# khanhha/temporal_inverse_kinematics

Measured on NVIDIA B200. Metric: IK-solved frames/sec (ST-GCN fwd + SMPL-X FK), higher is better.
Workload: dtype bf16

## Files before the change

include/tik.h:

```cpp
#ifndef TIK_H_
#define TIK_H_

#include <stdint.h>

#ifdef __cplusplus
extern "C" {
#endif

#define TIK_OK 0
#define TIK_ERR_INVALID (-1)
#define TIK_ERR_CUDA (-2)
#define TIK_ERR_UNSUPPORTED (-3)
#define TIK_ERR_WORKSPACE (-4)

#define TIK_F32 0
#define TIK_BF16 1

#define TIK_MAX_BLOCKS 16
#define TIK_MAX_SLABS 6
#define TIK_MAX_JOINTS 64

int tik_version(void);
const char* tik_last_error(void);
int tik_check_device(void);
// ... 16 lines not shown
int tik_stem_gcn(int dtype, const float* x_dev, const float* in_scale_dev, const float* in_shift_dev,
                 const float* agg_dev, const float* w_dev, const float* bias_dev, void* out_dev,
                 const float* res_w_dev, void* res_out_dev, int res_stride,
                 int64_t N, int T, int V, int Cin, int K, int Cout, int relu, void* stream);

typedef struct TikWindowing {
  int64_t frames;
  int32_t offset, stride, root_a, root_b;
} TikWindowing;

int tik_aggregate(int dtype, const void* x_dev, const float* agg_dev, void* out_dev,
                  int64_t N, int T, int V, int C, int K, void* stream);

int tik_gcn_fused(const void* x_dev, const void* abd_dev, const void* w_dev, const float* bias_dev, void* out_dev,
                  int64_t N, int T, int V, int Cin, int Cout, int relu, void* stream);

typedef struct TikSlab {
  const void* a_dev;
  int32_t c;
  int32_t t_in;
  int32_t t_mul;
  int32_t t_off;
} TikSlab;

#define TIK_ACT_NONE 0
#define TIK_ACT_RELU 1
#define TIK_ACT_LEAKY 2
#define TIK_RES_NONE 0
#define TIK_RES_IDENTITY 1
#define TIK_RES_STEM 2
// ... 127 lines not shown
```

temporal_inverse_kinematics_b200/_lib.py:

```python
import ctypes as C
import os

_HERE = os.path.dirname(os.path.abspath(__file__))
LIB_PATH = os.environ.get("TIK_LIB_PATH") or os.path.join(_HERE, "libtik.so")

HEADER_PATH = os.path.join(os.path.dirname(_HERE), "include", "tik.h")


def _header_defines():
    import re
    out = {}
    with open(HEADER_PATH) as f:
        for m in re.finditer(r"^#define\s+(TIK_\w+)\s+\(?(-?\d+)\)?", f.read(), re.M):
            out[m.group(1)] = int(m.group(2))
    return out


_H = _header_defines()
TIK_F32, TIK_BF16 = _H["TIK_F32"], _H["TIK_BF16"]
MAX_BLOCKS, MAX_SLABS, MAX_JOINTS = _H["TIK_MAX_BLOCKS"], _H["TIK_MAX_SLABS"], _H["TIK_MAX_JOINTS"]
ACT_NONE, ACT_RELU, ACT_LEAKY = 0, 1, 2
RES_NONE, RES_IDENTITY, RES_STEM, RES_CONV = 0, 1, 2, 3
OUT_NODE_MAJOR, OUT_TIME_MAJOR, OUT_ROWS_F32 = 0, 1, 2

# ... 49 lines not shown
    "tik_last_error": (C.c_char_p, []),
    "tik_check_device": (C.c_int, []),
    "tik_rot6d_to_rotmat": (C.c_int, [vp, vp, i64, vp]),
    "tik_aa_to_rotmat": (C.c_int, [vp, vp, i64, vp]),
    "tik_batch_rodrigues": (C.c_int, [vp, vp, i64, vp]),
    "tik_rotmat_to_aa": (C.c_int, [vp, vp, i64, C.c_int, vp]),
    "tik_quat_to_rotmat": (C.c_int, [vp, vp, i64, vp]),
    "tik_rotmat_to_quat": (C.c_int, [vp, vp, i64, vp]),
    "tik_quat_to_aa": (C.c_int, [vp, vp, i64, vp]),
    "tik_fk_body": (C.c_int, [vp, C.c_int, C.POINTER(f32), C.POINTER(i32), C.c_int, vp, vp, vp, vp, i64, vp]),
    "tik_stem_gcn": (C.c_int, [C.c_int, vp, vp, vp, vp, vp, vp, vp, vp, vp, C.c_int, i64, C.c_int, C.c_int, C.c_int,
                               C.c_int, C.c_int, C.c_int, vp]),
    "tik_aggregate": (C.c_int, [C.c_int, vp, vp, vp, i64, C.c_int, C.c_int, C.c_int, C.c_int, vp]),
    "tik_rowgemm": (C.c_int, [C.c_int, C.POINTER(TikRowGemm), vp]),
    "tik_gcn_fused": (C.c_int, [vp, vp, vp, vp, vp, i64, C.c_int, C.c_int, C.c_int, C.c_int, C.c_int, vp]),
    "tik_pack_bn": (C.c_int, [C.POINTER(TikRawBN), i64, vp, vp, vp]),
    "tik_pack_block_bytes": (C.c_int, [C.POINTER(TikRawBlock), C.c_int, C.c_int, C.POINTER(i64)]),
    "tik_pack_block": (C.c_int, [C.POINTER(TikRawBlock), C.c_int, C.c_int, C.POINTER(TikRawBN), C.POINTER(TikPackBuffers),
                                 C.POINTER(TikBlock), vp]),
    "tik_stgcn_out_frames": (C.c_int, [C.POINTER(TikNet), C.c_int]),
    "tik_stgcn_workspace_bytes": (C.c_int, [C.POINTER(TikNet), C.c_int, i64, i64, C.c_int, C.POINTER(i64)]),
    "tik_stgcn_plan_create": (C.c_int, [C.POINTER(TikNet), C.c_int, i64, i64, C.c_int, vp, i64, C.POINTER(vp)]),
    "tik_stgcn_plan_run": (C.c_int, [vp, vp, i64, vp, vp, vp]),
    "tik_stgcn_plan_run_windows": (C.c_int, [vp, vp, C.POINTER(TikWindowing), i64, vp, vp, vp]),
    "tik_stgcn_plan_profile": (C.c_int, [vp, vp, i64, vp, vp, C.POINTER(C.c_double), C.POINTER(i64), C.POINTER(C.c_double)]),
    "tik_stgcn_plan_launches": (i64, [vp, i64]),
    "tik_stgcn_plan_destroy": (None, [vp]),
    "tik_stgcn_latency_workspace_bytes": (C.c_int, [C.POINTER(TikNet), i64, C.c_int, C.POINTER(i64)]),
    "tik_stgcn_latency_create": (C.c_int, [C.POINTER(TikNet), i64, C.c_int, vp, i64, C.POINTER(vp)]),
    "tik_stgcn_latency_run": (C.c_int, [vp, vp, i64, vp, vp]),
# ... 63 lines not shown
```

temporal_inverse_kinematics_b200/build.py:

```python
import os
import shutil
import subprocess
import sys

HERE = os.path.dirname(os.path.abspath(__file__))
CSRC = os.path.join(HERE, "csrc")
LIB = os.path.join(HERE, "libtik.so")
SOURCES = ["geometry.cu", "fk.cu", "stem.cu", "stem_block.cu", "stgcn_simt.cu", "rowgemm_tf32.cu", "stgcn_umma.cu", "gcn_fused.cu", "tcn_halo.cu", "plan.cu", "latency.cu", "pack.cu"]
HEADERS = ["tik_common.cuh", "umma_prepared.h", "umma_ptx.cuh", os.path.join("..", "..", "include", "tik.h")]


def _nvcc():
    for c in (os.environ.get("NVCC"), shutil.which("nvcc"), "/usr/local/cuda/bin/nvcc"):
        if c and os.path.exists(c):
            return c
    raise RuntimeError("nvcc not found")


STAMP = os.path.join(HERE, "build", "flavour.txt")


def _flavour():
    if os.environ.get("TIK_TEST_WAIT") == "1":
        return "probe-testwait" if os.environ.get("TIK_PROBE") == "1" else "testwait"
# ... 58 lines not shown
```

temporal_inverse_kinematics_b200/csrc/plan.cu:

```cuda
#include <stdlib.h>
#include <string.h>

#include <algorithm>
#include <vector>

#include "tik_common.cuh"
#include "umma_prepared.h"

namespace tik {

static thread_local char g_err[512] = "";

bool pdl_enabled() {
  static int v = -1;
  if (v < 0) v = getenv("TIK_NO_PDL") ? 0 : 1;
  return v != 0;
}

LaunchOpts& launch_opts() {
  static thread_local LaunchOpts o = {0, 0};
  return o;
}
static int serpentine_enabled() {
  const char* e = getenv("TIK_SERPENTINE");
  return e ? atoi(e) : 1;
}
static int l2_hint_enabled() {
  const char* e = getenv("TIK_L2_HINT");
  return e ? atoi(e) : 0;
}

void set_error(const char* fmt, ...) {
  va_list ap;
  va_start(ap, fmt);
  vsnprintf(g_err, sizeof(g_err), fmt, ap);
  va_end(ap);
}

static int out_frames(int t, int stride) { return (t - 1) / stride + 1; }
static int64_t align_up(int64_t v, int64_t a) { return (v + a - 1) / a * a; }

struct Step {
  enum Kind { STEM = 0, AGG = 1, GEMM = 2, FUSED_GCN = 3, STEM_BLOCK = 4, TCN_HALO = 5 } kind;
  GcnFusedPrepared* fused = nullptr;
  StemBlockPrepared* stem_block = nullptr;
  TcnHaloPrepared* halo = nullptr;
  double fused_flops_per_clip = 0;
  TikRowGemm g;
  UmmaPrepared* prep = nullptr;
  const void* src = nullptr;
  void* dst = nullptr;
  void* dst2 = nullptr;
  int t = 0, c = 0;
  const TikBlock* blk = nullptr;
  bool out_is_feat = false;
  bool out_is_poses = false;
  bool agg_only = false;
  int k_identity = 0;
  const float* w_big = nullptr;
  const float* w_small = nullptr;
};
// ... 6 lines not shown
  int64_t n_chunk, n_max;
  int T, T_out;
  size_t es;
  std::vector<tik::Step> chunk_steps, batch_steps;
  uint8_t* feat = nullptr;
  int64_t feat_elems_per_clip = 0;
  int c_last = 0;
  ~TikPlan() {
    for (auto* v : {&chunk_steps, &batch_steps})
      for (auto& s : *v)
      {
        if (s.prep) tik::umma_free(s.prep);
        if (s.fused) tik::gcn_fused_free(s.fused);
        if (s.stem_block) tik::stem_block_free(s.stem_block);
        if (s.halo) tik::tcn_halo_free(s.halo);
      }
  }
};

namespace tik {

struct WsLayout {
  int64_t off_x0, off_x1, off_agg, off_h, off_r0, off_feat, off_z, off_abd, off_w16, off_eye, off_zbias, off_wsplit, total_bytes;
};

static int check_net(const TikNet* net, int dtype) {
  TIK_CHECK_ARG(net != nullptr, "null net");
  TIK_CHECK_ARG(dtype == TIK_F32 || dtype == TIK_BF16, "bad dtype %d", dtype);
  TIK_CHECK_ARG(net->n_blocks >= 1 && net->n_blocks <= TIK_MAX_BLOCKS, "n_blocks=%d", net->n_blocks);
  TIK_CHECK_ARG(net->V >= 1 && net->V <= 32 && net->K >= 1 && net->K <= 5, "V=%d K=%d unsupported", net->V, net->K);
// ... 55 lines not shown
  L->off_zbias = off; off = align_up(off + 32 * 128 * 4, 1024);
  L->off_wsplit = off;
  if (dtype == TIK_F32) {
    int64_t w_elems = 0;
    for (int i = 0; i < net->n_blocks; ++i) {
      const TikBlock& b = net->blocks[i];
      if (b.c_out <= 64) w_elems += align_up((int64_t)b.c_out * net->K * b.c_in, 256) + align_up((int64_t)b.c_out * (b.kt * b.c_out + b.c_in), 256);
    }
    if (net->head_hidden > 0 && net->head_hidden <= 64) w_elems += align_up((int64_t)net->head_hidden * V * net->blocks[net->n_blocks - 1].c_out, 256);
    if (net->head_hidden > 0 && net->head_out <= 64) w_elems += align_up((int64_t)net->head_out * net->head_hidden, 256);
    off = align_up(off + 2 * w_elems * 4, 1024);
  }
  L->total_bytes = off;
}

static int run_step(TikPlan* P, Step& st, const float* xc, int64_t n, int64_t clip_off, float* poses, cudaStream_t s,
                    const TikWindowing* win = nullptr, int64_t win_n0 = 0) {
  const TikNet& net = P->net;
  const int V = net.V;
  if (st.kind == Step::STEM) {
    const TikBlock& b = *st.blk;
    return stem_gcn_impl(P->dtype, xc, net.in_scale_dev, net.in_shift_dev, b.agg_dev, reinterpret_cast<const float*>(b.w_gcn_dev),
                         b.b_gcn_dev, st.dst, st.dst2 ? b.w_res_stem_dev : nullptr, st.dst2, b.stride, n, st.t, V, b.c_in, net.K,
                         b.c_out, 1, win, win_n0, s);
  }
  if (st.kind == Step::AGG) {
    return tik_aggregate(P->dtype, st.src, st.blk->agg_dev, st.dst, P->n_chunk, st.t, V, st.c, net.K, s);
  }
  if (st.kind == Step::FUSED_GCN) return gcn_fused_launch(st.fused, n, s);
  if (st.kind == Step::STEM_BLOCK) return stem_block_launch(st.stem_block, xc, n, win, win_n0, s);
  if (st.kind == Step::TCN_HALO) return tcn_halo_launch(st.halo, n * V, s);
  TikRowGemm g = st.g;
  if (g.v == 1) {
    g.t_out = (int32_t)(n * P->T_out);
    g.slabs[0].t_in = g.t_out;
  } else {
    g.nv = n * V;
  }
  if (st.out_is_feat) g.out_dev = P->feat + clip_off * P->feat_elems_per_clip * (int64_t)P->es;
  if (st.out_is_poses) g.out_dev = poses;
  return P->dtype == TIK_BF16 ? umma_launch(st.prep, &g, s) : rowgemm_f32_presplit(&g, st.w_big, st.w_small, s);
}

static int run_impl(TikPlan* P, const float* x, int64_t N, float* poses, void* feat_out, cudaStream_t s,
                    std::vector<cudaEvent_t>* events, std::vector<std::pair<Step*, int64_t>>* trace,
                    const TikWindowing* win = nullptr) {
// ... 114 lines not shown
  for (int i = 0; i < net->n_blocks; ++i) {
    const TikBlock& b = P->net.blocks[i];
    const int pad = (b.kt - 1) / 2;
    const int t_o = out_frames(t, b.stride);
    const bool last = i == net->n_blocks - 1;
    if (i == 0 && net->n_blocks > 1 && stem_block_supported(net, dtype) && !getenv("TIK_NO_STEM_BLOCK")) {
      Step s; s.kind = Step::STEM_BLOCK; s.blk = &b; s.t = t;
      int rcs = stem_block_prepare(&P->net, ws + L.off_w16, xbuf[0], n_chunk, t, &s.stem_block);
      if (rcs != TIK_OK) { delete P; return rcs; }
      s.fused_flops_per_clip = 2.0 * V * t * (double)b.c_out * (K * b.c_in + b.kt * b.c_out + (b.res_kind == TIK_RES_STEM ? b.c_in : 0));
      P->chunk_steps.push_back(s);
      cur = 0;
      t = t_o;
      continue;
    }
    if (i == 0) {
      Step s; s.kind = Step::STEM; s.dst = hbuf; s.t = t; s.blk = &b;
      s.dst2 = b.res_kind == TIK_RES_STEM ? r0buf : nullptr;
      P->chunk_steps.push_back(s);
    } else if (dtype == TIK_BF16 && gcn_fused_supported(b.c_in, b.c_out, V, K) && !getenv("TIK_NO_FUSED_GCN")) {
      const int f = gcn_fused_frames(t, b.c_in);
      std::vector<float> a_host((size_t)V * V);
      cudaError_t ce = cudaMemcpy(a_host.data(), b.agg_dev, a_host.size() * sizeof(float), cudaMemcpyDeviceToHost);
      std::vector<__nv_bfloat16> abd_host(128 * 128, __float2bfloat16_rn(0.f));
      for (int w = 0; w < V; ++w)
        for (int v = 0; v < V; ++v)
          for (int q = 0; q < f; ++q) abd_host[(size_t)(w * f + q) * 128 + (v * f + q)] = __float2bfloat16_rn(a_host[(size_t)v * V + w]);
      void* abd_dev = ws + L.off_abd + (int64_t)i * 128 * 128 * 2;
      if (ce == cudaSuccess) ce = cudaMemcpy(abd_dev, abd_host.data(), abd_host.size() * 2, cudaMemcpyHostToDevice);
      if (ce != cudaSuccess) { set_error("plan: Abd upload failed: %s", cudaGetErrorString(ce)); delete P; return TIK_ERR_CUDA; }
      Step s; s.kind = Step::FUSED_GCN; s.blk = &b; s.t = t;
      int rcf = gcn_fused_prepare(xbuf[cur], abd_dev, b.w_gcn_dev, b.b_gcn_dev, hbuf, n_chunk, t, V, b.c_in, b.c_out, 1, &s.fused);
      if (rcf != TIK_OK) { delete P; return rcf; }
      s.fused_flops_per_clip = 2.0 * V * t * (double)b.c_in * b.c_out;
      P->chunk_steps.push_back(s);
    } else {
      const bool tc_agg = dtype == TIK_BF16 && K == 1 && b.c_in % 128 == 0 && gcn_fused_supported(128, 128, V, 1) &&
                          !getenv("TIK_NO_FUSED_GCN") && !getenv("TIK_NO_TC_AGG");
      if (tc_agg) {
        const int f = gcn_fused_frames(t);
        std::vector<float> a_host((size_t)V * V);
        cudaError_t ce = cudaMemcpy(a_host.data(), b.agg_dev, a_host.size() * sizeof(float), cudaMemcpyDeviceToHost);
        std::vector<__nv_bfloat16> abd_host(128 * 128, __float2bfloat16_rn(0.f)), eye_host(128 * 128, __float2bfloat16_rn(0.f));
        for (int w = 0; w < V; ++w)
          for (int v = 0; v < V; ++v)
            for (int q = 0; q < f; ++q) abd_host[(size_t)(w * f + q) * 128 + (v * f + q)] = __float2bfloat16_rn(a_host[(size_t)v * V + w]);
        for (int d = 0; d < 128; ++d) eye_host[(size_t)d * 128 + d] = __float2bfloat16_rn(1.f);
        void* abd_dev = ws + L.off_abd + (int64_t)i * 128 * 128 * 2;
        if (ce == cudaSuccess) ce = cudaMemcpy(abd_dev, abd_host.data(), abd_host.size() * 2, cudaMemcpyHostToDevice);
        if (ce == cudaSuccess) ce = cudaMemcpy(ws + L.off_eye, eye_host.data(), eye_host.size() * 2, cudaMemcpyHostToDevice);
        if (ce == cudaSuccess) ce = cudaMemset(ws + L.off_zbias, 0, 32 * 128 * 4);
        if (ce != cudaSuccess) { set_error("plan: aggregation operands upload failed: %s", cudaGetErrorString(ce)); delete P; return TIK_ERR_CUDA; }
        for (int c0 = 0; c0 < b.c_in; c0 += 128) {
          Step s; s.kind = Step::FUSED_GCN; s.blk = &b; s.t = t; s.agg_only = true;
          int rcf = gcn_fused_prepare(reinterpret_cast<uint8_t*>(xbuf[cur]) + (size_t)c0 * 2, abd_dev, ws + L.off_eye,
                                      reinterpret_cast<const float*>(ws + L.off_zbias), reinterpret_cast<uint8_t*>(agg) + (size_t)c0 * 2,
                                      n_chunk, t, V, 128, 128, 0, &s.fused, b.c_in, b.c_in);
          if (rcf != TIK_OK) { delete P; return rcf; }
          P->chunk_steps.push_back(s);
        }
      } else {
        Step s; s.kind = Step::AGG; s.src = xbuf[cur]; s.dst = agg; s.t = t; s.c = b.c_in; s.blk = &b;
        P->chunk_steps.push_back(s);
      }
// ... 125 lines not shown
  TIK_CHECK_ARG(P->net.head_hidden == 0 || poses, "poses pointer required");
  std::vector<cudaEvent_t> ev;
  std::vector<std::pair<Step*, int64_t>> trace;
  cudaStream_t s = (cudaStream_t)stream;
  int rc = run_impl(P, x, N, poses, nullptr, s, &ev, &trace);
  if (rc != TIK_OK) return rc;
  TIK_CUDA(cudaStreamSynchronize(s));
  for (int k = 0; k < 3; ++k) { ms_by_kind[k] = 0; launches_by_kind[k] = 0; }
  *flops_gemm = 0;
  for (size_t i = 0; i < trace.size(); ++i) {
    float ms = 0;
    TIK_CUDA(cudaEventElapsedTime(&ms, ev[i], ev[i + 1]));
    Step& st = *trace[i].first;
    const int64_t n = trace[i].second;
    const int kind = st.agg_only ? (int)Step::AGG
                     : (st.kind == Step::FUSED_GCN || st.kind == Step::STEM_BLOCK || st.kind == Step::TCN_HALO) ? (int)Step::GEMM : (int)st.kind;
    ms_by_kind[kind] += ms;
    launches_by_kind[kind] += 1;
    if (getenv("TIK_PLAN_TRACE")) {
      static const char* names[] = {"stem", "aggregate", "gemm", "fused_gcn", "stem_block", "tcn_halo"};
      int ktot = 0;
      for (int q = 0; q < st.g.n_slabs && st.kind == Step::GEMM; ++q) ktot += st.g.slabs[q].c;
      fprintf(stderr, "tik trace: step %2zu %-9s clips=%lld K=%d c_out=%d t_out=%d  %.1f us\n", i, names[st.kind], (long long)n, ktot,
              st.kind == Step::GEMM ? st.g.c_out : st.c, st.kind == Step::GEMM ? st.g.t_out : st.t, ms * 1e3);
    }
    if (st.kind == Step::FUSED_GCN || st.kind == Step::STEM_BLOCK || st.kind == Step::TCN_HALO) *flops_gemm += st.fused_flops_per_clip * (double)n;
    if (st.kind == Step::GEMM) {
      double ktot = -st.k_identity;
      for (int q = 0; q < st.g.n_slabs; ++q) ktot += st.g.slabs[q].c;
      const double rows = st.g.v == 1 ? (double)n * P->T_out : (double)n * P->net.V * st.g.t_out;
      *flops_gemm += 2.0 * rows * ktot * st.g.c_out_valid;
    }
  }
  for (auto e : ev) cudaEventDestroy(e);
  return TIK_OK;
}

int64_t tik_stgcn_plan_launches(const TikPlan* P, int64_t N) {
  if (!P || N <= 0) return 0;
  int64_t total = 0;
  for (int64_t b0 = 0; b0 < N; b0 += P->n_max) {
// ... 10 lines not shown
```

temporal_inverse_kinematics_b200/csrc/umma_prepared.h:

```cpp
#pragma once
#include <cuda.h>
#include <cuda_runtime.h>
#include <stdint.h>

#include "../../include/tik.h"

namespace tik {
struct UmmaPrepared;
int umma_prepare(const TikRowGemm* d, int64_t nv_capacity, UmmaPrepared** out);
int umma_launch(UmmaPrepared* u, const TikRowGemm* d, cudaStream_t s);
void umma_free(UmmaPrepared* u);
struct GcnFusedPrepared;
bool gcn_fused_supported(int cin, int cout, int V, int K);
int gcn_fused_frames(int T);
int gcn_fused_frames(int T, int cin);
int gcn_fused_prepare(const void* x, const void* abd, const void* w, const float* bias, void* out, int64_t n_clips, int T, int V,
                      int cin, int cout, int relu, GcnFusedPrepared** outp, int x_row = 0, int out_row = 0);
int gcn_fused_launch(GcnFusedPrepared* g, int64_t n_clips, cudaStream_t s);
void gcn_fused_free(GcnFusedPrepared* g);
int encode_bf16_map(CUtensorMap* m, const void* base, int rank, const uint64_t* dims, const uint64_t* strides, const uint32_t* box);
struct StemBlockPrepared;
bool stem_block_supported(const TikNet* net, int dtype);
int64_t stem_block_workspace_bytes();
int stem_block_prepare(const TikNet* net, void* w16_dev, void* out, int64_t n_clips, int T, StemBlockPrepared** outp);
int stem_block_launch(StemBlockPrepared* g, const float* x, int64_t n_clips, const TikWindowing* win, int64_t win_n0, cudaStream_t s);
void stem_block_free(StemBlockPrepared* g);
struct TcnHaloPrepared;
bool tcn_halo_supported(int c, int c_out, int kt, int stride, int T, bool identity_slab);
int tcn_halo_prepare(const void* h, const void* x, const void* w, const float* bias, void* out, int64_t nv_cap, int T, int c,
                     TcnHaloPrepared** outp);
int tcn_halo_launch(TcnHaloPrepared* g, int64_t nv, cudaStream_t s);
void tcn_halo_free(TcnHaloPrepared* g);
}
```

temporal_inverse_kinematics_b200/ops.py:

```python
import ctypes as C

import torch

from . import _lib as L


def _code(t):
    if t.dtype == torch.float32:
        return L.TIK_F32
    if t.dtype == torch.bfloat16:
        return L.TIK_BF16
    raise TypeError(f"unsupported activation dtype {t.dtype}")


def _dev(*ts):
    for t in ts:
        if t is not None and not t.is_cuda:
            raise RuntimeError("libtik ops need CUDA tensors -- there is no CPU fallback")
        if t is not None and not t.is_contiguous():
            raise ValueError("libtik ops need contiguous tensors")


def to_node_major(x_nctv, dtype):
    return x_nctv.permute(0, 3, 2, 1).to(dtype).contiguous()
# ... 37 lines not shown
    abd[: V * f, : V * f] = torch.kron(a.t().contiguous(), torch.eye(f, device=A_hat.device))
    return abd.to(torch.bfloat16).contiguous()


def gcn_fused(x, abd, w, bias, relu=True):
    _dev(x, abd, w, bias)
    N, V, T, Cin = x.shape
    Cout = w.shape[0]
    out = torch.empty((N, V, T, Cout), dtype=torch.bfloat16, device=x.device)
    with L.on_device(x):
        L.check(L.lib().tik_gcn_fused(L.ptr(x), L.ptr(abd), L.ptr(w), L.ptr(bias), L.ptr(out), N, T, V, Cin, Cout, int(relu),
                                      L.stream_ptr(x.device)))
    return out


def rowgemm(slabs, w, bias, nv, v, t_out, act="none", slope=0.01, residual=None, out_layout="node", c_out_valid=None,
            stem_residual=None, out=None):
    a0 = slabs[0][0]
    _dev(w, bias, residual, *[s[0] for s in slabs])
    code = _code(a0)
    g = L.TikRowGemm()
    g.n_slabs = len(slabs)
    for i, (a, t_mul, t_off) in enumerate(slabs):
        if a.dtype != a0.dtype:
            raise TypeError("all slabs must share one dtype")
        g.slabs[i].a_dev = a.data_ptr()
        g.slabs[i].c = a.shape[-1]
        g.slabs[i].t_in = a.shape[-2]
        g.slabs[i].t_mul, g.slabs[i].t_off = t_mul, t_off
    c_out = w.shape[0]
# ... 36 lines not shown
```

Baseline: 69.09 million.

## Fuse whole 64-channel ST-GCN block into one warp-specialized UMMA kernel

Adds a persistent tcgen05/TMEM kernel that does the graph aggregation, the GCN GEMM with bias and ReLU, the 3-tap temporal conv, and the identity residual with ReLU for 64-channel stride-1 blocks. It runs as a single plan step in place of the separate fused-GCN and TCN-halo launches. The intermediate activation stays in shared memory and TMEM instead of going through global memory. TMA loads, MMAs and epilogues are pipelined with mbarriers. Costs are a complex synchronization scheme, and the temporal halo overlap recomputes some frames at tile edges.

```diff
diff --git a/include/tik.h b/include/tik.h
--- a/include/tik.h
+++ b/include/tik.h
@@ -54,6 +54,9 @@
 
 int tik_gcn_fused(const void* x_dev, const void* abd_dev, const void* w_dev, const float* bias_dev, void* out_dev,
                   int64_t N, int T, int V, int Cin, int Cout, int relu, void* stream);
+
+int tik_block_fused(const void* x_dev, const void* abd_dev, const void* wg_dev, const float* bias1_dev, const void* wt_dev,
+                    const float* bias2_dev, void* out_dev, int64_t N, int T, int V, int C, void* stream);
 
 typedef struct TikSlab {
   const void* a_dev;
diff --git a/temporal_inverse_kinematics_b200/_lib.py b/temporal_inverse_kinematics_b200/_lib.py
--- a/temporal_inverse_kinematics_b200/_lib.py
+++ b/temporal_inverse_kinematics_b200/_lib.py
@@ -87,6 +87,7 @@
     "tik_aggregate": (C.c_int, [C.c_int, vp, vp, vp, i64, C.c_int, C.c_int, C.c_int, C.c_int, vp]),
     "tik_rowgemm": (C.c_int, [C.c_int, C.POINTER(TikRowGemm), vp]),
     "tik_gcn_fused": (C.c_int, [vp, vp, vp, vp, vp, i64, C.c_int, C.c_int, C.c_int, C.c_int, C.c_int, vp]),
+    "tik_block_fused": (C.c_int, [vp, vp, vp, vp, vp, vp, vp, i64, C.c_int, C.c_int, C.c_int, vp]),
     "tik_pack_bn": (C.c_int, [C.POINTER(TikRawBN), i64, vp, vp, vp]),
     "tik_pack_block_bytes": (C.c_int, [C.POINTER(TikRawBlock), C.c_int, C.c_int, C.POINTER(i64)]),
     "tik_pack_block": (C.c_int, [C.POINTER(TikRawBlock), C.c_int, C.c_int, C.POINTER(TikRawBN), C.POINTER(TikPackBuffers),
diff --git a/temporal_inverse_kinematics_b200/build.py b/temporal_inverse_kinematics_b200/build.py
--- a/temporal_inverse_kinematics_b200/build.py
+++ b/temporal_inverse_kinematics_b200/build.py
@@ -6,7 +6,7 @@
 HERE = os.path.dirname(os.path.abspath(__file__))
 CSRC = os.path.join(HERE, "csrc")
 LIB = os.path.join(HERE, "libtik.so")
-SOURCES = ["geometry.cu", "fk.cu", "stem.cu", "stem_block.cu", "stgcn_simt.cu", "rowgemm_tf32.cu", "stgcn_umma.cu", "gcn_fused.cu", "tcn_halo.cu", "plan.cu", "latency.cu", "pack.cu"]
+SOURCES = ["geometry.cu", "fk.cu", "stem.cu", "stem_block.cu", "stgcn_simt.cu", "rowgemm_tf32.cu", "stgcn_umma.cu", "gcn_fused.cu", "tcn_halo.cu", "block_fused.cu", "plan.cu", "latency.cu", "pack.cu"]
 HEADERS = ["tik_common.cuh", "umma_prepared.h", "umma_ptx.cuh", os.path.join("..", "..", "include", "tik.h")]
 
 
diff --git a/temporal_inverse_kinematics_b200/csrc/block_fused.cu b/temporal_inverse_kinematics_b200/csrc/block_fused.cu
--- /dev/null
+++ b/temporal_inverse_kinematics_b200/csrc/block_fused.cu
@@ -0,0 +1,429 @@
+#include <string.h>
+
+#include <algorithm>
+
+#include "tik_common.cuh"
+#include "umma_prepared.h"
+#include "umma_ptx.cuh"
+
+namespace tik {
+
+constexpr int kBfG = kBlockFusedGroupFrames;
+constexpr int kBfF = 2 * kBfG;
+constexpr int kBfLoMax = kBfF - 2;
+constexpr int kBfC = 64;
+constexpr int kBfMaxV = 128 / kBfG;
+constexpr int kBfGroupWarps = 8;
+constexpr int kBfThreads = 96 + 2 * 32 * kBfGroupWarps;
+constexpr int kBfTile = 16384;
+constexpr int kBfXBufs = 3;
+constexpr int kBfHBytes = 1024 + 2 * kBfTile + 1024;
+constexpr int kBfBiasLd = kBfC + 4;
+constexpr int kBfOffWg = 0;
+constexpr int kBfOffWt = kBfOffWg + 8192;
+constexpr int kBfOffX = kBfOffWt + 3 * 8192;
+constexpr int kBfOffH = kBfOffX + kBfXBufs * 2 * kBfTile;
+constexpr int kBfOffBias1 = kBfOffH + 2 * kBfHBytes;
+constexpr int kBfOffBias2 = kBfOffBias1 + kBfMaxV * kBfBiasLd * 4;
+constexpr int kBfOffBar = kBfOffBias2 + kBfC * 4;
+constexpr int kBfSmemBytes = kBfOffBar + 256 + 1024;
+
+struct BlockFusedParams {
+  CUtensorMap map_x, map_out, map_wg, map_wt;
+  const __nv_bfloat16* abd;
+  const float* bias1;
+  const float* bias2;
+  int32_t n_clips, T, V, lo, tiles_t;
+  int32_t rev;
+};
+
+template <int C>
+__global__ void __launch_bounds__(kBfThreads, 1) block_fused_kernel(const __grid_constant__ BlockFusedParams p) {
+  static_assert(C == kBfC, "64-channel blocks only");
+  extern __shared__ uint8_t smem_raw[];
+  uint8_t* smem = smem_raw + ((1024u - (smem_u32(smem_raw) & 1023u)) & 1023u);
+  uint8_t* s_wg = smem + kBfOffWg;
+  uint8_t* s_wt = smem + kBfOffWt;
+  uint8_t* s_x = smem + kBfOffX;
+  uint8_t* s_h = smem + kBfOffH;
+  float* s_bias1 = reinterpret_cast<float*>(smem + kBfOffBias1);
+  float* s_bias2 = reinterpret_cast<float*>(smem + kBfOffBias2);
+  uint64_t* bars = reinterpret_cast<uint64_t*>(smem + kBfOffBar);
+  uint64_t* w_full = bars;
+  uint64_t* x_full = bars + 1;
+  uint64_t* x_empty = bars + 4;
+  uint64_t* d1_full = bars + 7;
+  uint64_t* xagg_full = bars + 8;
+  uint64_t* d2_full = bars + 9;
+  uint64_t* h_full = bars + 11;
+  uint64_t* d3_full = bars + 13;
+  uint64_t* tmem_empty = bars + 15;
+  uint64_t* stage_full = bars + 17;
+  uint64_t* h_empty = bars + 19;
+  uint32_t* tmem_slot = reinterpret_cast<uint32_t*>(bars + 21);
+
+  const int warp = threadIdx.x >> 5, lane = threadIdx.x & 31;
+  const int V = p.V;
+  const int n_tiles = p.n_clips * p.tiles_t;
+  const int my_tiles = n_tiles > (int)blockIdx.x ? (n_tiles - (int)blockIdx.x + (int)gridDim.x - 1) / (int)gridDim.x : 0;
+  const int rows_valid = kBfG * V;
+
+  if (warp == 0 && lane == 0) {
+    tma_prefetch_desc(&p.map_x); tma_prefetch_desc(&p.map_out); tma_prefetch_desc(&p.map_wg); tma_prefetch_desc(&p.map_wt);
+  }
+  if (warp == 1 && lane == 0) {
+    mbar_init(w_full, 1);
+    for (int i = 0; i < kBfXBufs; ++i) { mbar_init(&x_full[i], 1); mbar_init(&x_empty[i], kBfGroupWarps); }
+    mbar_init(d1_full, 1); mbar_init(xagg_full, kBfGroupWarps);
+    for (int i = 0; i < 2; ++i) {
+      mbar_init(&d2_full[i], 1); mbar_init(&h_full[i], kBfGroupWarps); mbar_init(&d3_full[i], 1);
+      mbar_init(&tmem_empty[i], kBfGroupWarps); mbar_init(&stage_full[i], kBfGroupWarps); mbar_init(&h_empty[i], 1);
+    }
+    fence_barrier_init();
+  }
+  if (warp == 2) tmem_alloc<512>(tmem_slot);
+  for (int i = threadIdx.x; i < V * C; i += kBfThreads) s_bias1[(i / C) * kBfBiasLd + (i % C)] = __ldg(p.bias1 + i);
+  for (int i = threadIdx.x; i < C; i += kBfThreads) s_bias2[i] = __ldg(p.bias2 + i);
+  {
+    const int pad_rows = 128 - rows_valid;
+    const int total16 = kBfXBufs * 2 * pad_rows * 8;
+    for (int i = threadIdx.x; i < total16; i += kBfThreads) {
+      const int piece = i & 7, rr = (i >> 3) % pad_rows, slab = (i >> 3) / pad_rows;
+      *reinterpret_cast<uint4*>(s_x + (size_t)slab * kBfTile + (size_t)(rows_valid + rr) * 128 + piece * 16) = make_uint4(0, 0, 0, 0);
+    }
+    fence_proxy_async_smem();
+  }
+  tc_fence_before();
+  __syncthreads();
+  tc_fence_after();
+  const uint32_t tmem_base = *tmem_slot;
+  const uint32_t tmem_abd = tmem_base, tmem_d1 = tmem_base + 64, tmem_d2 = tmem_base + 192;
+  if (warp >= 3 && warp < 7) {
+    const int r = (warp & 3) * 32 + lane;
+    const uint4* arow = reinterpret_cast<const uint4*>(p.abd + (size_t)r * 128);
+    uint4 v[16];
+#pragma unroll
+    for (int u = 0; u < 16; ++u) v[u] = __ldg(arow + u);
+#pragma unroll
+    for (int u = 0; u < 8; ++u) {
+      const uint32_t w8[8] = {v[2 * u].x, v[2 * u].y, v[2 * u].z, v[2 * u].w, v[2 * u + 1].x, v[2 * u + 1].y, v[2 * u + 1].z, v[2 * u + 1].w};
+      tmem_st8(tmem_abd + ((uint32_t)((warp & 3) * 32) << 16) + (uint32_t)(8 * u), w8);
+    }
+    tmem_st_wait();
+  }
+  tc_fence_before();
+  __syncthreads();
+  tc_fence_after();
+  pdl_launch_dependents();
+  pdl_wait();
+
+  auto tile_of = [&](int it, int& n, int& tt) {
+    const int tile = (int)blockIdx.x + it * (int)gridDim.x;
+    const int nf = tile / p.tiles_t;
+    tt = tile - nf * p.tiles_t;
+    n = p.rev ? p.n_clips - 1 - nf : nf;
+  };
+
+  if (warp == 0) {
+    if (lane == 0) {
+      mbar_expect_tx(w_full, (uint32_t)(4 * 8192));
+      tma_load_2d(s_wg, &p.map_wg, w_full, 0, 0);
+      for (int dt = 0; dt < 3; ++dt) tma_load_2d(s_wt + dt * 8192, &p.map_wt, w_full, dt * C, 0);
+      for (int it = 0; it < my_tiles; ++it) {
+        int n, tt;
+        tile_of(it, n, tt);
+        const int xb = it % kBfXBufs;
+        mbar_wait(&x_empty[xb], (uint32_t)(((it / kBfXBufs) & 1) ^ 1));
+        mbar_expect_tx(&x_full[xb], (uint32_t)(2 * rows_valid * 128));
+        const int t_first = tt * p.lo - 1;
+        for (int g = 0; g < 2; ++g)
+          tma_load_4d(s_x + (size_t)(xb * 2 + g) * kBfTile, &p.map_x, &x_full[xb], 0, t_first + kBfG * g, 0, n);
+      }
+    }
+  } else if (warp == 1) {
+    constexpr uint32_t idesc1 = make_idesc_bf16(128, 128) | (1u << 16);
+    constexpr uint32_t idesc = make_idesc_bf16(128, C);
+    const bool leader = lane == 0;
+    mbar_wait(w_full, 0);
+    const uint32_t wg_u32 = smem_u32(s_wg), wt_u32 = smem_u32(s_wt), x_u32 = smem_u32(s_x), h_u32 = smem_u32(s_h);
+    auto issue_mma1 = [&](int it) {
+      const int xb = it % kBfXBufs;
+      mbar_wait(&x_full[xb], (uint32_t)((it / kBfXBufs) & 1));
+      tc_fence_after();
+      if (leader) {
+        const uint32_t xaddr = x_u32 + (uint32_t)(xb * 2) * kBfTile;
+#pragma unroll
+        for (int k = 0; k < 8; ++k)
+          umma_bf16_ts(tmem_d1, tmem_abd + (uint32_t)(8 * k), make_smem_desc_mnmajor_sw128(xaddr + (uint32_t)k * 2048u, (uint32_t)kBfTile),
+                       idesc1, k != 0 ? 1u : 0u);
+        umma_commit(d1_full);
+      }
+      __syncwarp();
+    };
+    auto issue_mma2 = [&](int it) {
+      const int s = it & 1;
+      mbar_wait(xagg_full, (uint32_t)(it & 1));
+      mbar_wait(&tmem_empty[s], (uint32_t)(((it >> 1) & 1) ^ 1));
+      tc_fence_after();
+      if (leader) {
+#pragma unroll
+        for (int g = 0; g < 2; ++g)
+#pragma unroll
+          for (int k = 0; k < 4; ++k)
+            umma_bf16_ts(tmem_d2 + (uint32_t)(s * 128 + g * 64), tmem_d1 + (uint32_t)(g * 64 + k * 8),
+                         make_smem_desc_kmajor_sw128(wg_u32 + (uint32_t)k * 32u), idesc, k != 0 ? 1u : 0u);
+        umma_commit(&d2_full[s]);
+      }
+      __syncwarp();
+    };
+    if (my_tiles > 0) { issue_mma1(0); issue_mma2(0); }
+    for (int it = 0; it < my_tiles; ++it) {
+      const int s = it & 1;
+      const uint32_t par = (uint32_t)((it >> 1) & 1);
+      const uint32_t dcol = tmem_d2 + (uint32_t)(s * 128);
+      if (it + 1 < my_tiles) { issue_mma1(it + 1); issue_mma2(it + 1); }
+      mbar_wait(&h_full[s], par);
+      tc_fence_after();
+      if (leader) {
+        const uint32_t hb = h_u32 + (uint32_t)s * kBfHBytes + 1024u;
+#pragma unroll
+        for (int dt = 0; dt < 3; ++dt)
+#pragma unroll
+          for (int j = 0; j < 2; ++j) {
+            const uint32_t arow = hb + (uint32_t)(128 * j + dt - 1) * 128u;
+#pragma unroll
+            for (int k = 0; k < 4; ++k)
+              umma_bf16(dcol + (uint32_t)(j * 64), make_smem_desc_kmajor_sw128(arow + (uint32_t)k * 32u),
+                        make_smem_desc_kmajor_sw128(wt_u32 + (uint32_t)dt * 8192u + (uint32_t)k * 32u), idesc, (dt | k) != 0 ? 1u : 0u);
+          }
+        umma_commit(&d3_full[s]);
+      }
+      __syncwarp();
+    }
+  } else if (warp == 2) {
+    if (lane == 0) {
+      for (int it = 0; it < my_tiles; ++it) {
+        const int s = it & 1;
+        int n, tt;
+        tile_of(it, n, tt);
+        mbar_wait(&stage_full[s], (uint32_t)((it >> 1) & 1));
+        tma_store_4d(&p.map_out, s_h + (size_t)s * kBfHBytes + 1024, 0, tt * p.lo, 0, n);
+        tma_store_commit();
+        tma_store_wait_read0();
+        mbar_arrive(&h_empty[s]);
+      }
+      tma_store_wait0();
+    }
+  } else if (warp < 3 + kBfGroupWarps) {
+    const int lane_grp = warp & 3;
+    const int g = (warp - 3) >> 2;
+    const int r = lane_grp * 32 + lane;
+    const uint32_t lane_off = (uint32_t)(lane_grp * 32) << 16;
+    const int v = r / kBfG, l = kBfG * g + (r - v * kBfG);
+    const bool row_ok = v < V;
+    const int hrow = v * kBfF + l;
+    const float* bias = s_bias1 + (row_ok ? v : 0) * kBfBiasLd;
+    auto convert = [&](int it) {
+      mbar_wait(d1_full, (uint32_t)(it & 1));
+      tc_fence_after();
+#pragma unroll
+      for (int c = 0; c < 2; ++c) {
+        uint32_t a[32];
+        tmem_ld16(tmem_d1 + lane_off + (uint32_t)(g * 64 + 32 * c), a);
+        tmem_ld16(tmem_d1 + lane_off + (uint32_t)(g * 64 + 32 * c + 16), a + 16);
+        tmem_ld_wait();
+#pragma unroll
+        for (int q = 0; q < 2; ++q) {
+          uint32_t w8[8];
+#pragma unroll
+          for (int e = 0; e < 8; ++e) w8[e] = pack_bf16x2(__uint_as_float(a[16 * q + 2 * e]), __uint_as_float(a[16 * q + 2 * e + 1]));
+          tmem_st8(tmem_d1 + lane_off + (uint32_t)(g * 64 + 16 * c + 8 * q), w8);
+        }
+      }
+      tmem_st_wait();
+      tc_fence_before();
+      __syncwarp();
+      if (lane == 0) mbar_arrive(xagg_full);
+    };
+    if (my_tiles > 0) convert(0);
+    for (int it = 0; it < my_tiles; ++it) {
+      const int s = it & 1;
+      const uint32_t par = (uint32_t)((it >> 1) & 1);
+      int n, tt;
+      tile_of(it, n, tt);
+      const int t = tt * p.lo - 1 + l;
+      const bool ok = row_ok && t >= 0 && t < p.T;
+      mbar_wait(&d2_full[s], par);
+      tc_fence_after();
+      mbar_wait(&h_empty[s], par ^ 1);
+      uint8_t* hb = s_h + (size_t)s * kBfHBytes + 1024;
+#pragma unroll
+      for (int c = 0; c < 2; ++c) {
+        uint32_t a[32];
+        tmem_ld16(tmem_d2 + lane_off + (uint32_t)(s * 128 + g * 64 + 32 * c), a);
+        tmem_ld16(tmem_d2 + lane_off + (uint32_t)(s * 128 + g * 64 + 32 * c + 16), a + 16);
+        tmem_ld_wait();
+        if (row_ok) {
+#pragma unroll
+          for (int q = 0; q < 4; ++q) {
+            const float4 b0 = *reinterpret_cast<const float4*>(bias + 32 * c + 8 * q);
+            const float4 b1 = *reinterpret_cast<const float4*>(bias + 32 * c + 8 * q + 4);
+            uint4 u;
+            u.x = pack_bf16x2_relu(__uint_as_float(a[8 * q + 0]) + b0.x, __uint_as_float(a[8 * q + 1]) + b0.y);
+            u.y = pack_bf16x2_relu(__uint_as_float(a[8 * q + 2]) + b0.z, __uint_as_float(a[8 * q + 3]) + b0.w);
+            u.z = pack_bf16x2_relu(__uint_as_float(a[8 * q + 4]) + b1.x, __uint_as_float(a[8 * q + 5]) + b1.y);
+            u.w = pack_bf16x2_relu(__uint_as_float(a[8 * q + 6]) + b1.z, __uint_as_float(a[8 * q + 7]) + b1.w);
+            if (!ok) u = make_uint4(0, 0, 0, 0);
+            *reinterpret_cast<uint4*>(hb + (size_t)hrow * 128 + (((4 * c + q) ^ (hrow & 7)) << 4)) = u;
+          }
+        }
+      }
+      tc_fence_before();
+      fence_proxy_async_smem();
+      __syncwarp();
+      if (lane == 0) mbar_arrive(&h_full[s]);
+      if (it + 1 < my_tiles) convert(it + 1);
+    }
+  } else {
+    const int lane_grp = warp & 3;
+    const int half = (warp - 3 - kBfGroupWarps) >> 2;
+    const int i_row = lane_grp * 32 + lane;
+    const uint32_t lane_off = (uint32_t)(lane_grp * 32) << 16;
+    float bias[32];
+#pragma unroll
+    for (int e = 0; e < 32; ++e) bias[e] = s_bias2[half * 32 + e];
+    for (int it = 0; it < my_tiles; ++it) {
+      const int s = it & 1;
+      const int xb = it % kBfXBufs;
+      mbar_wait(&d3_full[s], (uint32_t)((it >> 1) & 1));
+      tc_fence_after();
+      mbar_wait(&x_full[xb], (uint32_t)((it / kBfXBufs) & 1));
+      uint8_t* stage = s_h + (size_t)s * kBfHBytes + 1024;
+#pragma unroll
+      for (int j = 0; j < 2; ++j) {
+        uint32_t a[32];
+        tmem_ld16(tmem_d2 + lane_off + (uint32_t)(s * 128 + j * 64 + half * 32), a);
+        tmem_ld16(tmem_d2 + lane_off + (uint32_t)(s * 128 + j * 64 + half * 32 + 16), a + 16);
+        tmem_ld_wait();
+        if (j == 1) {
+          tc_fence_before();
+          __syncwarp();
+          if (lane == 0) mbar_arrive(&tmem_empty[s]);
+        }
+        const int h = 128 * j + i_row;
+        const int v = h / kBfF, l = h - v * kBfF;
+        if (v < V && l >= 1 && l <= p.lo) {
+          const int srow = v * p.lo + l - 1;
+          const int g = l >= kBfG ? 1 : 0;
+          const int xr = v * kBfG + l - kBfG * g;
+          const uint8_t* xrow = s_x + (size_t)(xb * 2 + g) * kBfTile + (size_t)xr * 128;
+#pragma unroll
+          for (int q = 0; q < 4; ++q) {
+            const uint4 xv = *reinterpret_cast<const uint4*>(xrow + (((half * 4 + q) ^ (xr & 7)) << 4));
+            const uint32_t xw[4] = {xv.x, xv.y, xv.z, xv.w};
+            uint32_t o[4];
+#pragma unroll
+            for (int e = 0; e < 4; ++e) {
+              const float2 xf = __bfloat1622float2(*reinterpret_cast<const __nv_bfloat162*>(&xw[e]));
+              o[e] = pack_bf16x2_relu(__uint_as_float(a[8 * q + 2 * e]) + bias[8 * q + 2 * e] + xf.x,
+                                      __uint_as_float(a[8 * q + 2 * e + 1]) + bias[8 * q + 2 * e + 1] + xf.y);
+            }
+            *reinterpret_cast<uint4*>(stage + (size_t)srow * 128 + (((half * 4 + q) ^ (srow & 7)) << 4)) = make_uint4(o[0], o[1], o[2], o[3]);
+          }
+        }
+      }
+      fence_proxy_async_smem();
+      __syncwarp();
+      if (lane == 0) { mbar_arrive(&stage_full[s]); mbar_arrive(&x_empty[xb]); }
+    }
+  }
+  __syncwarp();
+  tc_fence_before();
+  __syncthreads();
+  if (warp == 2) {
+    tc_fence_after();
+    tmem_dealloc<512>(tmem_base);
+  }
+}
+
+struct BlockFusedPrepared {
+  BlockFusedParams p;
+  int64_t cap;
+};
+
+bool block_fused_supported(int c_in, int c_out, int V, int K) { return K == 1 && c_in == kBfC && c_out == kBfC && V >= 1 && V <= kBfMaxV; }
+
+int block_fused_prepare(const void* x, const void* abd, const void* wg, const float* bias1, const void* wt, int wt_k,
+                        const float* bias2, void* out, int64_t n_clips, int T, int V, int c, BlockFusedPrepared** outp) {
+  TIK_CHECK_ARG(block_fused_supported(c, c, V, 1), "fused block: unsupported shape c=%d V=%d", c, V);
+  TIK_CHECK_ARG(x && abd && wg && bias1 && wt && bias2 && out && n_clips > 0 && T > 0 && wt_k >= 3 * c, "fused block: bad arguments");
+  BlockFusedPrepared* g = new BlockFusedPrepared();
+  BlockFusedParams& p = g->p;
+  memset(&p, 0, sizeof(p));
+  g->cap = n_clips;
+  p.abd = reinterpret_cast<const __nv_bfloat16*>(abd);
+  p.bias1 = bias1; p.bias2 = bias2;
+  p.n_clips = (int32_t)n_clips; p.T = T; p.V = V;
+  p.lo = T < kBfLoMax ? T : kBfLoMax;
+  p.tiles_t = (T + p.lo - 1) / p.lo;
+  TIK_CHECK_ARG(n_clips * p.tiles_t < (1ll << 31), "fused block: too many tiles");
+  int rc;
+  {
+    uint64_t dims[4] = {(uint64_t)c, (uint64_t)T, (uint64_t)V, (uint64_t)n_clips};
+    uint64_t strides[3] = {(uint64_t)c * 2, (uint64_t)c * 2 * T, (uint64_t)c * 2 * T * V};
+    uint32_t box[4] = {64, (uint32_t)kBfG, (uint32_t)V, 1};
+    rc = encode_bf16_map(&p.map_x, x, 4, dims, strides, box);
+    uint32_t obox[4] = {64, (uint32_t)p.lo, (uint32_t)V, 1};
+    if (rc == TIK_OK) rc = encode_bf16_map(&p.map_out, out, 4, dims, strides, obox);
+  }
+  if (rc == TIK_OK) {
+    uint64_t dims[2] = {(uint64_t)c, (uint64_t)c};
+    uint64_t strides[1] = {(uint64_t)c * 2};
+    uint32_t box[2] = {64, (uint32_t)c};
+    rc = encode_bf16_map(&p.map_wg, wg, 2, dims, strides, box);
+  }
+  if (rc == TIK_OK) {
+    uint64_t dims[2] = {(uint64_t)wt_k, (uint64_t)c};
+    uint64_t strides[1] = {(uint64_t)wt_k * 2};
+    uint32_t box[2] = {64, (uint32_t)c};
+    rc = encode_bf16_map(&p.map_wt, wt, 2, dims, strides, box);
+  }
+  if (rc != TIK_OK) { delete g; return rc; }
+  *outp = g;
+  return TIK_OK;
+}
+
+int block_fused_launch(BlockFusedPrepared* g, int64_t n_clips, cudaStream_t s) {
+  TIK_CHECK_ARG(g && n_clips <= g->cap, "fused block: n_clips exceeds the prepared capacity");
+  if (n_clips <= 0) return TIK_OK;
+  BlockFusedParams p = g->p;
+  p.n_clips = (int32_t)n_clips;
+  p.rev = launch_opts().rev;
+  static bool attr_done[64] = {};
+  int dev = 0;
+  TIK_CUDA(cudaGetDevice(&dev));
+  if (!attr_done[dev & 63]) {
+    TIK_CUDA(cudaFuncSetAttribute(block_fused_kernel<kBfC>, cudaFuncAttributeMaxDynamicSharedMemorySize, kBfSmemBytes));
+    attr_done[dev & 63] = true;
+  }
+  int sms = 148;
+  cudaDeviceGetAttribute(&sms, cudaDevAttrMultiProcessorCount, dev);
+  const unsigned grid = (unsigned)std::min<int64_t>(n_clips * p.tiles_t, sms);
+  TIK_CUDA(launch_pdl(block_fused_kernel<kBfC>, grid, kBfThreads, (size_t)kBfSmemBytes, s, p));
+  return TIK_OK;
+}
+
+void block_fused_free(BlockFusedPrepared* g) { delete g; }
+
+}
+
+extern "C" int tik_block_fused(const void* x_dev, const void* abd_dev, const void* wg_dev, const float* bias1_dev, const void* wt_dev,
+                               const float* bias2_dev, void* out_dev, int64_t N, int T, int V, int C, void* stream) {
+  using namespace tik;
+  BlockFusedPrepared* g = nullptr;
+  int rc = block_fused_prepare(x_dev, abd_dev, wg_dev, bias1_dev, wt_dev, 3 * C, bias2_dev, out_dev, N, T, V, C, &g);
+  if (rc != TIK_OK) return rc;
+  rc = block_fused_launch(g, N, (cudaStream_t)stream);
+  block_fused_free(g);
+  return rc;
+}
diff --git a/temporal_inverse_kinematics_b200/csrc/plan.cu b/temporal_inverse_kinematics_b200/csrc/plan.cu
--- a/temporal_inverse_kinematics_b200/csrc/plan.cu
+++ b/temporal_inverse_kinematics_b200/csrc/plan.cu
@@ -24,6 +24,10 @@
 static int serpentine_enabled() {
   const char* e = getenv("TIK_SERPENTINE");
   return e ? atoi(e) : 1;
+}
+static bool fused_block_enabled() {
+  const char* e = getenv("TIK_NO_FUSED_BLOCK");
+  return !(e && atoi(e) != 0);
 }
 static int l2_hint_enabled() {
   const char* e = getenv("TIK_L2_HINT");
@@ -41,10 +45,11 @@
 static int64_t align_up(int64_t v, int64_t a) { return (v + a - 1) / a * a; }
 
 struct Step {
-  enum Kind { STEM = 0, AGG = 1, GEMM = 2, FUSED_GCN = 3, STEM_BLOCK = 4, TCN_HALO = 5 } kind;
+  enum Kind { STEM = 0, AGG = 1, GEMM = 2, FUSED_GCN = 3, STEM_BLOCK = 4, TCN_HALO = 5, FUSED_BLOCK = 6 } kind;
   GcnFusedPrepared* fused = nullptr;
   StemBlockPrepared* stem_block = nullptr;
   TcnHaloPrepared* halo = nullptr;
+  BlockFusedPrepared* block = nullptr;
   double fused_flops_per_clip = 0;
   TikRowGemm g;
   UmmaPrepared* prep = nullptr;
@@ -81,6 +86,7 @@
         if (s.fused) tik::gcn_fused_free(s.fused);
         if (s.stem_block) tik::stem_block_free(s.stem_block);
         if (s.halo) tik::tcn_halo_free(s.halo);
+        if (s.block) tik::block_fused_free(s.block);
       }
   }
 };
@@ -166,6 +172,17 @@
   L->total_bytes = off;
 }
 
+static cudaError_t upload_abd(const TikBlock& b, int V, int f, void* abd_dev) {
+  std::vector<float> a_host((size_t)V * V);
+  cudaError_t ce = cudaMemcpy(a_host.data(), b.agg_dev, a_host.size() * sizeof(float), cudaMemcpyDeviceToHost);
+  if (ce != cudaSuccess) return ce;
+  std::vector<__nv_bfloat16> abd_host(128 * 128, __float2bfloat16_rn(0.f));
+  for (int w = 0; w < V; ++w)
+    for (int v = 0; v < V; ++v)
+      for (int q = 0; q < f; ++q) abd_host[(size_t)(w * f + q) * 128 + (v * f + q)] = __float2bfloat16_rn(a_host[(size_t)v * V + w]);
+  return cudaMemcpy(abd_dev, abd_host.data(), abd_host.size() * 2, cudaMemcpyHostToDevice);
+}
+
 static int run_step(TikPlan* P, Step& st, const float* xc, int64_t n, int64_t clip_off, float* poses, cudaStream_t s,
                     const TikWindowing* win = nullptr, int64_t win_n0 = 0) {
   const TikNet& net = P->net;
@@ -182,6 +199,7 @@
   if (st.kind == Step::FUSED_GCN) return gcn_fused_launch(st.fused, n, s);
   if (st.kind == Step::STEM_BLOCK) return stem_block_launch(st.stem_block, xc, n, win, win_n0, s);
   if (st.kind == Step::TCN_HALO) return tcn_halo_launch(st.halo, n * V, s);
+  if (st.kind == Step::FUSED_BLOCK) return block_fused_launch(st.block, n, s);
   TikRowGemm g = st.g;
   if (g.v == 1) {
     g.t_out = (int32_t)(n * P->T_out);
@@ -326,20 +344,30 @@
       t = t_o;
       continue;
     }
+    if (dtype == TIK_BF16 && i > 0 && !last && b.res_kind == TIK_RES_IDENTITY && b.kt == 3 && b.stride == 1 &&
+        block_fused_supported(b.c_in, b.c_out, V, K) && fused_block_enabled() && !getenv("TIK_NO_FUSED_GCN") &&
+        !getenv("TIK_NO_TCN_HALO")) {
+      void* abd_dev = ws + L.off_abd + (int64_t)i * 128 * 128 * 2;
+      const cudaError_t ce = upload_abd(b, V, kBlockFusedGroupFrames, abd_dev);
+      if (ce != cudaSuccess) { set_error("plan: Abd upload failed: %s", cudaGetErrorString(ce)); delete P; return TIK_ERR_CUDA; }
+      const int nxt = cur ^ 1;
+      Step s; s.kind = Step::FUSED_BLOCK; s.blk = &b; s.t = t; s.c = b.c_out;
+      int rcb = block_fused_prepare(xbuf[cur], abd_dev, b.w_gcn_dev, b.b_gcn_dev, b.w_tcn_dev, b.kt * b.c_out + (b.res_as_slab ? b.c_out : 0),
+                                    b.b_tcn_dev, xbuf[nxt], n_chunk, t, V, b.c_out, &s.block);
+      if (rcb != TIK_OK) { delete P; return rcb; }
+      s.fused_flops_per_clip = 2.0 * V * t * (double)b.c_out * (K * b.c_in + b.kt * b.c_out);
+      P->chunk_steps.push_back(s);
+      cur = nxt;
+      t = t_o;
+      continue;
+    }
     if (i == 0) {
       Step s; s.kind = Step::STEM; s.dst = hbuf; s.t = t; s.blk = &b;
       s.dst2 = b.res_kind == TIK_RES_STEM ? r0buf : nullptr;
       P->chunk_steps.push_back(s);
     } else if (dtype == TIK_BF16 && gcn_fused_supported(b.c_in, b.c_out, V, K) && !getenv("TIK_NO_FUSED_GCN")) {
-      const int f = gcn_fused_frames(t, b.c_in);
-      std::vector<float> a_host((size_t)V * V);
-      cudaError_t ce = cudaMemcpy(a_host.data(), b.agg_dev, a_host.size() * sizeof(float), cudaMemcpyDeviceToHost);
-      std::vector<__nv_bfloat16> abd_host(128 * 128, __float2bfloat16_rn(0.f));
-      for (int w = 0; w < V; ++w)
-        for (int v = 0; v < V; ++v)
-          for (int q = 0; q < f; ++q) abd_host[(size_t)(w * f + q) * 128 + (v * f + q)] = __float2bfloat16_rn(a_host[(size_t)v * V + w]);
       void* abd_dev = ws + L.off_abd + (int64_t)i * 128 * 128 * 2;
-      if (ce == cudaSuccess) ce = cudaMemcpy(abd_dev, abd_host.data(), abd_host.size() * 2, cudaMemcpyHostToDevice);
+      const cudaError_t ce = upload_abd(b, V, gcn_fused_frames(t, b.c_in), abd_dev);
       if (ce != cudaSuccess) { set_error("plan: Abd upload failed: %s", cudaGetErrorString(ce)); delete P; return TIK_ERR_CUDA; }
       Step s; s.kind = Step::FUSED_GCN; s.blk = &b; s.t = t;
       int rcf = gcn_fused_prepare(xbuf[cur], abd_dev, b.w_gcn_dev, b.b_gcn_dev, hbuf, n_chunk, t, V, b.c_in, b.c_out, 1, &s.fused);
@@ -350,16 +378,10 @@
       const bool tc_agg = dtype == TIK_BF16 && K == 1 && b.c_in % 128 == 0 && gcn_fused_supported(128, 128, V, 1) &&
                           !getenv("TIK_NO_FUSED_GCN") && !getenv("TIK_NO_TC_AGG");
       if (tc_agg) {
-        const int f = gcn_fused_frames(t);
-        std::vector<float> a_host((size_t)V * V);
-        cudaError_t ce = cudaMemcpy(a_host.data(), b.agg_dev, a_host.size() * sizeof(float), cudaMemcpyDeviceToHost);
-        std::vector<__nv_bfloat16> abd_host(128 * 128, __float2bfloat16_rn(0.f)), eye_host(128 * 128, __float2bfloat16_rn(0.f));
-        for (int w = 0; w < V; ++w)
-          for (int v = 0; v < V; ++v)
-            for (int q = 0; q < f; ++q) abd_host[(size_t)(w * f + q) * 128 + (v * f + q)] = __float2bfloat16_rn(a_host[(size_t)v * V + w]);
+        std::vector<__nv_bfloat16> eye_host(128 * 128, __float2bfloat16_rn(0.f));
         for (int d = 0; d < 128; ++d) eye_host[(size_t)d * 128 + d] = __float2bfloat16_rn(1.f);
         void* abd_dev = ws + L.off_abd + (int64_t)i * 128 * 128 * 2;
-        if (ce == cudaSuccess) ce = cudaMemcpy(abd_dev, abd_host.data(), abd_host.size() * 2, cudaMemcpyHostToDevice);
+        cudaError_t ce = upload_abd(b, V, gcn_fused_frames(t), abd_dev);
         if (ce == cudaSuccess) ce = cudaMemcpy(ws + L.off_eye, eye_host.data(), eye_host.size() * 2, cudaMemcpyHostToDevice);
         if (ce == cudaSuccess) ce = cudaMemset(ws + L.off_zbias, 0, 32 * 128 * 4);
         if (ce != cudaSuccess) { set_error("plan: aggregation operands upload failed: %s", cudaGetErrorString(ce)); delete P; return TIK_ERR_CUDA; }
@@ -515,17 +537,18 @@
     Step& st = *trace[i].first;
     const int64_t n = trace[i].second;
     const int kind = st.agg_only ? (int)Step::AGG
-                     : (st.kind == Step::FUSED_GCN || st.kind == Step::STEM_BLOCK || st.kind == Step::TCN_HALO) ? (int)Step::GEMM : (int)st.kind;
+                     : (st.kind == Step::FUSED_GCN || st.kind == Step::STEM_BLOCK || st.kind == Step::TCN_HALO || st.kind == Step::FUSED_BLOCK)
+                         ? (int)Step::GEMM : (int)st.kind;
     ms_by_kind[kind] += ms;
     launches_by_kind[kind] += 1;
     if (getenv("TIK_PLAN_TRACE")) {
-      static const char* names[] = {"stem", "aggregate", "gemm", "fused_gcn", "stem_block", "tcn_halo"};
+      static const char* names[] = {"stem", "aggregate", "gemm", "fused_gcn", "stem_block", "tcn_halo", "fused_block"};
       int ktot = 0;
       for (int q = 0; q < st.g.n_slabs && st.kind == Step::GEMM; ++q) ktot += st.g.slabs[q].c;
       fprintf(stderr, "tik trace: step %2zu %-9s clips=%lld K=%d c_out=%d t_out=%d  %.1f us\n", i, names[st.kind], (long long)n, ktot,
               st.kind == Step::GEMM ? st.g.c_out : st.c, st.kind == Step::GEMM ? st.g.t_out : st.t, ms * 1e3);
     }
-    if (st.kind == Step::FUSED_GCN || st.kind == Step::STEM_BLOCK || st.kind == Step::TCN_HALO) *flops_gemm += st.fused_flops_per_clip * (double)n;
+    if (st.kind == Step::FUSED_GCN || st.kind == Step::STEM_BLOCK || st.kind == Step::TCN_HALO || st.kind == Step::FUSED_BLOCK) *flops_gemm += st.fused_flops_per_clip * (double)n;
     if (st.kind == Step::GEMM) {
       double ktot = -st.k_identity;
       for (int q = 0; q < st.g.n_slabs; ++q) ktot += st.g.slabs[q].c;
diff --git a/temporal_inverse_kinematics_b200/csrc/umma_prepared.h b/temporal_inverse_kinematics_b200/csrc/umma_prepared.h
--- a/temporal_inverse_kinematics_b200/csrc/umma_prepared.h
+++ b/temporal_inverse_kinematics_b200/csrc/umma_prepared.h
@@ -1,6 +1,7 @@
 #pragma once
 #include <cuda.h>
 #include <cuda_runtime.h>
+#include <cuda_bf16.h>
 #include <stdint.h>
 
 #include "../../include/tik.h"
@@ -31,4 +32,11 @@
                      TcnHaloPrepared** outp);
 int tcn_halo_launch(TcnHaloPrepared* g, int64_t nv, cudaStream_t s);
 void tcn_halo_free(TcnHaloPrepared* g);
+struct BlockFusedPrepared;
+bool block_fused_supported(int c_in, int c_out, int V, int K);
+constexpr int kBlockFusedGroupFrames = 7;
+int block_fused_prepare(const void* x, const void* abd, const void* wg, const float* bias1, const void* wt, int wt_k,
+                        const float* bias2, void* out, int64_t n_clips, int T, int V, int c, BlockFusedPrepared** outp);
+int block_fused_launch(BlockFusedPrepared* g, int64_t n_clips, cudaStream_t s);
+void block_fused_free(BlockFusedPrepared* g);
 }
diff --git a/temporal_inverse_kinematics_b200/ops.py b/temporal_inverse_kinematics_b200/ops.py
--- a/temporal_inverse_kinematics_b200/ops.py
+++ b/temporal_inverse_kinematics_b200/ops.py
@@ -75,6 +75,16 @@
     return out
 
 
+def block_fused(x, abd, wg, bias1, wt, bias2):
+    _dev(x, abd, wg, bias1, wt, bias2)
+    N, V, T, C = x.shape
+    out = torch.empty_like(x)
+    with L.on_device(x):
+        L.check(L.lib().tik_block_fused(L.ptr(x), L.ptr(abd), L.ptr(wg), L.ptr(bias1), L.ptr(wt), L.ptr(bias2), L.ptr(out),
+                                        N, T, V, C, L.stream_ptr(x.device)))
+    return out
+
+
 def rowgemm(slabs, w, bias, nv, v, t_out, act="none", slope=0.01, residual=None, out_layout="node", c_out_valid=None,
             stem_residual=None, out=None):
     a0 = slabs[0][0]
```

New measurement: 71.52 million, median of 6. +3.5%, better.
